# TimoLassmann/tagdust

Hardware: AMD Instinct MI355X
Metric: reads/s (150 bp, 8-barcode arch) (higher is better)
Workload: dtype f32

## Files before the change

tagdust_amd/csrc/td_jit.h:

```cpp
#pragma once
#include <string>
#include <vector>
#include "../../include/tagdust_hip.h"
#include "td_device.h"

#ifndef TD_HIDDEN
#define TD_HIDDEN __attribute__((visibility("hidden")))
#endif

struct TdSpecKnobs {
	int block = 512;
	int min_waves = 4;
	int lsum_oob = 1;
	int rt_min = 16;
	int groupcols = 18;
	int groupcols_fwd = 12;
	int prune = 1;
	int prune_sfx = 1;
	int restart = -1;
	int firstseg = -1;
	int trie_sh = 2;
	int profile = 0;
	int prune_stats = -1;
	std::string extra_opts;
};
TdSpecKnobs td_spec_knobs(void);

#define TD_PRUNE_TABLES 16
#define TD_PRUNE_RESTART_MAX 4

struct TdSpecPlan {
	TdSpecKnobs k;
	int S = 0, H = 0, C = 0;
	std::vector<int> col_off, hmm_off;
	std::vector<int> group, group_f;
	std::vector<int> pure_last, drop_m;
	std::vector<int> bw_off;
	int64_t halves = 0;
	std::vector<int> rt, rt_b;
	std::vector<int> base;
	std::vector<float> hi, lo, nv;
	bool trie_on = false;
	int trie_sh = 1, trie_n_share = 0;
	std::vector<int> trie_ord;
	int first_n = 0;
	int prune_segs = 0;
	int sfx_first = 0;
	float prune_z = 0.0f;
	int restart = 0;
};
TdSpecPlan td_spec_plan(const td_model_desc* m, const TdSpecKnobs& k);
TD_HIDDEN std::string td_spec_model_section(const td_model_desc* m, const TdSpecPlan& p, int lsum_oob, int window);

float td_spec_prune_z(const td_model_desc* m, int n_seg, int sfx_first);
void td_spec_prune_tables(const td_model_desc* m, const TdSpecPlan& p, int lcap, int stride, std::vector<float>& tab);
void td_spec_layout(TdSpecLayout& L, const TdSpecPlan& p, int lmax);
int td_spec_compile(const td_model_desc* m, const TdSpecPlan& p, int lsum_oob, int window, std::vector<char>& code, std::string& log,
                    uint64_t* key_out = nullptr, bool key_only = false);
int td_spec_compiles_started(void);
```

tagdust_amd/csrc/td_spec_kernel.inc:

```

#ifndef TDS_BLOCK
#define TDS_BLOCK 512
#endif
#ifndef TDS_MIN_WAVES
#define TDS_MIN_WAVES 4
#endif
#define TDS_REG_H 32
#define TDS_WPB (TDS_BLOCK / TD_WAVE)
#define NEG_INF (-__builtin_inff())
#define DEV __device__ __forceinline__

#define MODE_GET_LABEL 1
#define MODE_ARCH_COMP 5
#define OUT_SUCCESS 0
#define OUT_ARCH_MISMATCH 1
#define OUT_TOO_SHORT 2
#define OUT_BAR_FINGER_NOT_FOUND 3
#define OUT_MATCHES_ARTIFACTS 5
#define OUT_LOW_COMPLEXITY 6
#define N_OUTCOME_SLOTS 8
#define TDS_DIAG(k) (N_OUTCOME_SLOTS + 256 + ((k) - 192))

#ifndef TDS_LSUM_OOB
#define TDS_LSUM_OOB 1
// ... 131 lines not shown
}

#ifndef TDS_PROFILE
#define TDS_PROFILE 0
#endif
#define TDS_PHASE(k) do { if (TDS_PROFILE) { const long long t_ = (long long)__builtin_readcyclecounter(); \
	if (lane == 0) atomicAdd(&ka.counters[TDS_DIAG(240 + (k))], (unsigned long long)(t_ - tprof)); tprof = t_; } } while (0)

#ifndef TDS_WINDOW
#define TDS_WINDOW 0
#endif
constexpr bool kMaskDP = TD_H - kFirstN <= TDS_REG_H;

struct Wv {
	uint32_t* pmask;
	int nwm;
	uint8_t* slot;
	int lane, len, lmax, tmax, tmin;
	float* bm;
	uint8_t* ba;
	int cut;
	int cutS;
	const float* wa;
	const float* wb;
	int sstop;
	int sstopS;
	const float* wc;
	const float* wd;
	mutable int bad;
	bool rb_on, rf_on;
	float* rs;
	float* hb;
	int rWf;
	int rW;
	const float* bwt;
	const float* fbs;
	unsigned long long* stats;
	long long* tprof;
	const float* ptab;
	int pstride;
	const float* qr;
	const float* pr;
};

#ifndef TDS_LATE_CS
#define TDS_LATE_CS 1
#endif
#ifndef TDS_PF_DIST
#define TDS_PF_DIST 4
#endif
#ifndef TDS_PF_COLS
#define TDS_PF_COLS 2
#endif
#ifndef TDS_LDP
#define TDS_LDP 2
#endif
#ifndef TDS_LDT
#define TDS_LDT 4
#endif
#ifndef TDS_SCAN_B
#define TDS_SCAN_B 8
#endif
#ifndef TDS_PRUNE_TT
#define TDS_PRUNE_TT (-88.0f)
#endif
#ifndef TDS_PRUNE_MARGIN
#define TDS_PRUNE_MARGIN 1
#endif
#ifndef TDS_PRUNE_BGAP
#define TDS_PRUNE_BGAP 5.0f
#endif
#ifndef TDS_PRUNE_STATS
#define TDS_PRUNE_STATS 0
#endif

constexpr int cmin(int a, int b) { return a < b ? a : b; }
constexpr int pf_dist(int cols, bool rt) { return (!rt && cols <= TDS_PF_COLS) ? TDS_PF_DIST : 1; }
template <int D> struct IC { static constexpr int v = D; };
constexpr bool label_leading(int h)
{
	for (int j = 0; j < kPruneSegs; j++) if (h >= kHmmOff[j] && h < kHmmOff[j] + kNHmm[j]) return true;
	return false;
}
template <int PD, int D, typename F>
DEV void ring_block(F& step, const int base)
{
	if constexpr (D < PD) { step(IC<D>{}, base + D); ring_block<PD, D + 1>(step, base); }
}
template <int PD, int D, typename F>
DEV void ring_rest(F& step, const int base, const int iend)
{
	if constexpr (D < PD - 1) { if (base + D <= iend) { step(IC<D>{}, base + D); ring_rest<PD, D + 1>(step, base, iend); } }
}

template <int J, bool RT>
DEV void bwd_row(const int fa, const float (&Mn)[kNCol[J]], const float (&In)[kNCol[J]], const float Pn,
                 const BaseMask& kc, const int c, const BaseMask& kx, const int xi, SV (&Mc)[kNCol[J]], SV (&Ic)[kNCol[J]])
{
#define EM(gcol, mask, xval) (RT ? emit_rt(kBase[colr + (gcol)], kHi[J], kLo[J], kNv[J], mask, xval) : EMIT_M(col0 + (gcol), mask))
	constexpr int NC = kNCol[J];
	constexpr int K = NC - 1;
	const int col0 = kColOff[J] + (RT ? 0 : fa) * NC;
	const int colr = kColOff[J] + fa * NC;
	(void)colr;
	SV Dp = sv_none();
	{
		const int q = col0 + K;
		const SV M = addc(sv(Pn), kCols[q].t[7]);
		SV I = addc(sv(Pn), kCols[q].t[8]);
		I = lsum(I, addv(addc(sv(Mn[K]), kCols[q].t[4]), EM(K, kc, c)));
		I = lsum(I, addv(addc(sv(In[K]), kCols[q].t[3]), EMIT_I(q, kc)));
		Mc[K] = M; Ic[K] = I;
	}
#pragma unroll
	for (int g = K - 1; g >= 0; --g) {
		const int q = col0 + g;
		const float epc = EM(g + 1, kc, c);
		const float eic = EMIT_I(q, kc);
		SV M = addc(addv(sv(Mn[g + 1]), epc), kCols[q].t[0]);
		SV I = addv(addc(sv(In[g]), kCols[q].t[3]), eic);
		lsum2(M, addc(sv(Pn), kCols[q].t[7]), I, addc(sv(Pn), kCols[q].t[8]));
		lsum2(M, addc(addv(sv(In[g]), eic), kCols[q].t[1]), I, addv(addc(sv(Mn[g + 1]), kCols[q].t[4]), epc));
		SV D = addc(Dp, kCols[q].t[5]);
		lsum2(M, addc(Dp, kCols[q].t[2]), D, addc(addv(Mc[g + 1], EM(g + 1, kx, xi)), kCols[q].t[6]));
		Mc[g] = M; Ic[g] = I; Dp = D;
	}
#undef EM
}

template <int J, bool RT, int GT, int GB>
DEV void bwd_cols(const int fa, const float (&Mn)[kNCol[J]], const float (&In)[kNCol[J]], const float Pn,
                  const BaseMask& kc, const int c, const BaseMask& kx, const int xi, SV (&Mc)[kNCol[J]], SV (&Ic)[kNCol[J]], SV& Dp)
{
#define EM(gcol, mask, xval) (RT ? emit_rt(kBase[colr + (gcol)], kHi[J], kLo[J], kNv[J], mask, xval) : EMIT_M(col0 + (gcol), mask))
	constexpr int NC = kNCol[J];
	constexpr int K = NC - 1;
	const int col0 = kColOff[J] + (RT ? 0 : fa) * NC;
	const int colr = kColOff[J] + fa * NC;
	(void)colr;
	if constexpr (GT == K) {
		const int q = col0 + K;
		const SV M = addc(sv(Pn), kCols[q].t[7]);
		SV I = addc(sv(Pn), kCols[q].t[8]);
		I = lsum(I, addv(addc(sv(Mn[K]), kCols[q].t[4]), EM(K, kc, c)));
		I = lsum(I, addv(addc(sv(In[K]), kCols[q].t[3]), EMIT_I(q, kc)));
		Mc[K] = M; Ic[K] = I;
		Dp = sv_none();
	}
#pragma unroll
	for (int g = (GT == K ? K - 1 : GT); g >= GB; --g) {
		const int q = col0 + g;
		const float epc = EM(g + 1, kc, c);
		const float eic = EMIT_I(q, kc);
		SV M = addc(addv(sv(Mn[g + 1]), epc), kCols[q].t[0]);
		SV I = addv(addc(sv(In[g]), kCols[q].t[3]), eic);
		lsum2(M, addc(sv(Pn), kCols[q].t[7]), I, addc(sv(Pn), kCols[q].t[8]));
		lsum2(M, addc(addv(sv(In[g]), eic), kCols[q].t[1]), I, addv(addc(sv(Mn[g + 1]), kCols[q].t[4]), epc));
		SV D = addc(Dp, kCols[q].t[5]);
		lsum2(M, addc(Dp, kCols[q].t[2]), D, addc(addv(Mc[g + 1], EM(g + 1, kx, xi)), kCols[q].t[6]));
		Mc[g] = M; Ic[g] = I; Dp = D;
	}
#undef EM
}

#ifndef TDS_RESTART
#define TDS_RESTART 0
// ... 579 lines not shown
		}
		hi0 = fminf(hi0 + (__logf((float)(t > 1 ? t : 1)) + 0.02f), w.fbs[t]);
	}
	float Mlo[NC], Mhi[NC], Ilo[NC], Ihi[NC];
#pragma unroll
	for (int g = 0; g < NC; g++) { Mlo[g] = NEG_INF; Ilo[g] = NEG_INF; Mhi[g] = hi0; Ihi[g] = hi0; }
	int gc = 0;
	int closed_at = -1;
	auto close_check = [&](const int steps_done) __attribute__((always_inline)) {
		if (gc < NC) {
			bool cl = true;
#pragma unroll
			for (int g = 0; g < NC; g++) if (g == gc) cl = same(si(Mlo[g], Mhi[g])) && same(si(Ilo[g], Ihi[g]));
			if (__builtin_amdgcn_ballot_w64(!cl) == 0) { gc++; if (gc == NC) closed_at = steps_done; }
		}
	};
	int c_n = codes[q_lo * TD_WAVE + w.lane];
	float Pm_n = P[(q_lo - 1) * TD_WAVE + w.lane];
	for (int i = q_lo; i < q_hi; ++i) {
		const int c = c_n;
		const float Pm = Pm_n;
		{
			const int ip = (i + 1 < q_hi) ? i + 1 : i;
			c_n = codes[ip * TD_WAVE + w.lane];
			Pm_n = P[(ip - 1) * TD_WAVE + w.lane];
		}
		close_check(i - q_lo); close_check(i - q_lo);
		fstair_dispatch<J, 0>(gc, Mlo, Mhi, Ilo, Ihi, Pm, mk_mask(c));
	}
	close_check(q_hi - q_lo); close_check(q_hi - q_lo);
	if (gc < NC) w.bad |= 32;
	if (TDS_PRUNE_STATS && w.lane == 0) {
		const int st = closed_at >= 0 ? closed_at : q_hi - q_lo;
		atomicAdd(&w.stats[TDS_DIAG(194)], (unsigned long long)st); atomicAdd(&w.stats[TDS_DIAG(195)], 1ull);
		atomicMax(&w.stats[TDS_DIAG(192)], (unsigned long long)st);
	}
	float* rs = w.rs + (int64_t)kColOff[J] * 2 * TD_WAVE + w.lane;
#pragma unroll
	for (int g = 0; g < NC; g++) { rs[(2 * g) * TD_WAVE] = Mlo[g]; rs[(2 * g + 1) * TD_WAVE] = Ilo[g]; }
}

template <int J, int NF, bool RT>
DEV void fwd_group(const Wv& w, const uint8_t* __restrict__ codes, const float* __restrict__ P,
                   float* __restrict__ Cs, const float* __restrict__ PB, const uint8_t* __restrict__ BW,
                   float* __restrict__ DP, float* __restrict__ TOTAL, const float b, const int f0)
{
	const bool first = (f0 == 0);
#define EM(gcol, mask, xval) (RT ? emit_rt(kBase[colr + (gcol)], kHi[J], kLo[J], kNv[J], mask, xval) : EMIT_M(col0 + (gcol), mask))
	constexpr int NC = kNCol[J];
	constexpr int K = NC - 1;
	constexpr bool pure = kPureLast[J] != 0;
	constexpr int NS = NC - kPureLast[J];
	constexpr int DM = kDropM[J];
	constexpr int NSF = NS - DM;
	constexpr int ROWH = 2 * NS - DM;
	constexpr int NQ = NSF / 2;
	constexpr int NT = NSF & 1;
	constexpr bool skip_live = LIVE(kSkip[J]);
	float Mp[NF][NC], Ip[NF][NC], tot[NF];
#pragma unroll
	for (int f = 0; f < NF; f++) {
		tot[f] = NEG_INF;
#pragma unroll
		for (int g = 0; g < NC; g++) { Mp[f][g] = NEG_INF; Ip[f][g] = NEG_INF; }
	}
	if (TDS_RESTART && J >= kSfxFirst && w.rf_on) {
		const float* rs = w.rs + (int64_t)kColOff[J] * 2 * TD_WAVE + w.lane;
#pragma unroll
		for (int g = 0; g < NC; g++) { Mp[0][g] = rs[(2 * g) * TD_WAVE]; Ip[0][g] = rs[(2 * g + 1) * TD_WAVE]; }
	}
	constexpr bool p_init = (J == 0);
	const bool resumed = TDS_RESTART && (J >= kSfxFirst) && w.rf_on;
	const int i0 = resumed ? w.sstop - (TD_S - 1 - J) * (w.rWf + 1) : 1;
	float Pm = p_init ? 0.0f : P[(i0 - 1) * TD_WAVE + w.lane];
	constexpr int PD = pf_dist(NF * NC, RT);
	const int pmax = (w.tmax >= 1) ? w.tmax : 1;
	int c_q[PD];
	float Pi_q[PD], cs_q[PD], pb_q[PD], bm_q[PD], ik_q[PD][NF];
	int ba_q[PD];
	float MB_q[PD][NF][NSF + 1], IB_q[PD][NF][NSF + 1];
	constexpr bool pb_init = (J == TD_S - 1);
#define PBR(pos) (pb_init ? (((pos) == w.len + 1) ? 0.0f : NEG_INF) : PB[(pos) * TD_WAVE + w.lane])
#define BWROW(f_, pos_) (BW + ((int64_t)kBwOff[kHmmOff[J] + f0 + (f_)] * w.lmax + (int64_t)((pos_) - 1) * ROWH) * (TD_WAVE * 4))
#define TDS_FWD_FILL(d, p_raw) { \
		const int p_ = ((p_raw) <= pmax) ? (p_raw) : pmax; \
		c_q[d] = codes[p_ * TD_WAVE + w.lane]; \
		Pi_q[d] = p_init ? NEG_INF : P[p_ * TD_WAVE + w.lane]; \
		if (!first) cs_q[d] = Cs[p_ * TD_WAVE + w.lane]; \
		if (pure) pb_q[d] = PBR(p_ + 1); \
		if (own_sum && !first) { bm_q[d] = w.bm[p_ * TD_WAVE + w.lane]; ba_q[d] = w.ba[p_ * TD_WAVE + w.lane]; } \
		const bool rows_ = !((J >= kSfxFirst) && p_ < w.sstop);    \
_Pragma("unroll") \
		for (int f = 0; f < NF; f++) { \
			if (DM && rows_) ik_q[d][f] = ld1(BWROW(f, p_) + NSF * (TD_WAVE * 8), w.lane); \
			if (PD > 1 && rows_) { \
_Pragma("unroll") \
				for (int q = 0; q < NQ; q++) { \
					MB_q[d][f][2 * q] = ldk(BWROW(f, p_) + q * (TD_WAVE * 16), w.lane, 16, 0); IB_q[d][f][2 * q] = ldk(BWROW(f, p_) + q * (TD_WAVE * 16), w.lane, 16, 1); \
					MB_q[d][f][2 * q + 1] = ldk(BWROW(f, p_) + q * (TD_WAVE * 16), w.lane, 16, 2); IB_q[d][f][2 * q + 1] = ldk(BWROW(f, p_) + q * (TD_WAVE * 16), w.lane, 16, 3); \
				} \
				if (NT) { MB_q[d][f][NSF - 1] = ldk(BWROW(f, p_) + NQ * (TD_WAVE * 16), w.lane, 8, 0); IB_q[d][f][NSF - 1] = ldk(BWROW(f, p_) + NQ * (TD_WAVE * 16), w.lane, 8, 1); } \
			} \
		} \
	}
	constexpr bool own_sum = (J == 0) && (kFirstN > 0);
	float lacc[NF];
	uint32_t mbits[NF];
#pragma unroll
	for (int f = 0; f < NF; f++) { lacc[f] = 0.0f; mbits[f] = 0u; }
#pragma unroll
	for (int d = 0; d < PD; d++) {
		cs_q[d] = NEG_INF; pb_q[d] = 0.0f; bm_q[d] = -1.0f; ba_q[d] = 0;
#pragma unroll
		for (int f = 0; f < NF; f++) ik_q[d][f] = NEG_INF;
		TDS_FWD_FILL(d, i0 + d)
	}

	const int iend = (J < kPruneSegs && w.cut < w.tmax) ? w.cut : w.tmax;
	const int itail = (J == kPruneSegs && kPruneSegs > 0) ? w.cut + 1 : w.tmax + 1;
	(void)itail;
	if (i0 > 1 && kMaskDP && !own_sum) {
#pragma unroll
		for (int f = 0; f < NF; f++) {
			if (w.lane == 0) for (int wd = 0; wd < ((i0 - 1) >> 5); wd++) w.pmask[(kHmmOff[J] + f0 + f) * w.nwm + wd] = 0u;
			mbits[f] = 0u;
		}
	}
	auto step_cs = [&](auto dtag, auto cstag, const int i) __attribute__((always_inline)) {
		constexpr int d_ = decltype(dtag)::v;
		constexpr bool want_cs = decltype(cstag)::v != 0;
		const int c = c_q[d_];
		const float Pi = Pi_q[d_];
		const float pb = pb_q[d_];
		SV cs; cs.v = cs_q[d_]; cs.z = RT ? false : first;
		float bm = bm_q[d_];
		int ba = ba_q[d_];
		f32x4 cb[NF][NQ + 1];
		f32x2 ct[NF];
		const bool sfx_skip = (J >= kSfxFirst) && i < w.sstop;
		float ik[NF];
#pragma unroll
		for (int f = 0; f < NF; f++) {
			if constexpr (PD == 1) {
				const uint8_t* bw = BW + ((int64_t)kBwOff[kHmmOff[J] + f0 + f] * w.lmax + (int64_t)(i - 1) * ROWH) * (TD_WAVE * 4);
				if (!sfx_skip) {
#pragma unroll
					for (int p = 0; p < NQ; p++) cb[f][p] = ld4(bw + p * (TD_WAVE * 16), w.lane);
					if (NT) ct[f] = ld2(bw + NQ * (TD_WAVE * 16), w.lane);
				}
			} else {
#pragma unroll
				for (int p = 0; p < NQ; p++) cb[f][p] = f32x4{ MB_q[d_][f][2 * p], IB_q[d_][f][2 * p], MB_q[d_][f][2 * p + 1], IB_q[d_][f][2 * p + 1] };
				if (NT) ct[f] = f32x2{ MB_q[d_][f][NSF - 1], IB_q[d_][f][NSF - 1] };
			}
			ik[f] = ik_q[d_][f];
		}
		TDS_FWD_FILL(d_, i + PD)
		const int dn_ = (d_ + 1) % PD;
		const int c_n = c_q[dn_];
		const float pb_n = pb_q[dn_];
		float ik_n[NF];
#pragma unroll
		for (int f = 0; f < NF; f++) ik_n[f] = ik_q[dn_][f];
		float lpost[NF];
#pragma unroll
		for (int f = 0; f < NF; f++) lpost[f] = NEG_INF;
		const bool tail = (J == kPruneSegs && kPruneSegs > 0) && i >= itail;
		if (i <= w.len) {
			const SV PmS = sv(tail ? NEG_INF : Pm);
			const SV PiS = sv(tail ? NEG_INF : Pi);
			const BaseMask kc = mk_mask(c);
#pragma unroll
			for (int f = 0; f < NF; f++) {
				const int col0 = kColOff[J] + (RT ? 0 : (f0 + f)) * NC;
				const int colr = kColOff[J] + (f0 + f) * NC;
				(void)colr;
				const int h = kHmmOff[J] + f0 + f;
				SV Mc[NC], Ic[NC];
				SV Dc = sv_none();
				const float ei0 = EMIT_I(col0, kc);
				{
					const int q = col0;
					const SV M = addv(addc(PmS, kCols[q].sM), EM(0, kc, c));
					SV I = addc(PmS, kCols[q].sI);
					if (tail && LIVE(kCols[q].sI)) {
						if (!(Ip[f][0] + kCols[q].t[3] >= uload(w.wa, i))) w.bad |= 1;
					}
					I = lsum(I, addc(sv(Ip[f][0]), kCols[q].t[3]));
					I = lsum(I, addc(sv(Mp[f][0]), kCols[q].t[1]));
					I = addv(I, ei0);
					if (want_cs) { cs = lsum(cs, addc(M, kCols[q].t[7])); cs = lsum(cs, addc(I, kCols[q].t[8])); }
					Mc[0] = M; Ic[0] = I;
				}
#pragma unroll
				for (int g = 1; g <= K; ++g) {
					const int q = col0 + g, qp = q - 1;
					SV M = addc(PmS, kCols[q].sM);
					SV I = addc(PmS, kCols[q].sI);
					lsum2(M, addc(sv(Mp[f][g - 1]), kCols[qp].t[0]), I, addc(sv(Ip[f][g]), kCols[q].t[3]));
					lsum2(M, addc(sv(Ip[f][g - 1]), kCols[qp].t[4]), I, addc(sv(Mp[f][g]), kCols[q].t[1]));
					SV D = addc(Mc[g - 1], kCols[qp].t[2]);
					lsum2(M, addc(Dc, kCols[qp].t[6]), D, addc(Dc, kCols[qp].t[5]));
					M = addv(M, EM(g, kc, c));
					I = addv(I, EMIT_I(q, kc));
					if (want_cs) { cs = lsum(cs, addc(M, kCols[q].t[7])); cs = lsum(cs, addc(I, kCols[q].t[8])); }
					Mc[g] = M; Ic[g] = I; Dc = D;
				}
				if (tail && skip_live) { if (!(cs.v >= uload(w.wb, i))) w.bad |= 2; }
				if (want_cs) cs = lsum(cs, addc(PiS, kSkip[J]));
				if (!sfx_skip) {
				float MB[NC], IB[NC];
#pragma unroll
				for (int p = 0; p < NQ; p++) {
					const f32x4 v = cb[f][p];
					MB[2 * p] = v.x; IB[2 * p] = v.y; MB[2 * p + 1] = v.z; IB[2 * p + 1] = v.w;
				}
				if (NT) { MB[NSF - 1] = ct[f].x; IB[NSF - 1] = ct[f].y; }
				if constexpr (DM != 0) {
					constexpr int g = K - 1;
					const int q = col0 + g;
					const bool nxt = i < w.len;
					const int cx = (i < w.tmax) ? c_n : 0;
					const BaseMask kn = mk_mask(cx);
					SV MnK = addc(sv(pb_n), kCols[col0 + K].t[7]);
					if (!MnK.z) MnK.v = nxt ? MnK.v : NEG_INF;
					const float InK = nxt ? ik_n[f] : NEG_INF;
					SV Mr = addc(addv(MnK, EM(K, kn, cx)), kCols[q].t[0]);
					Mr = lsum(Mr, addc(sv(pb), kCols[q].t[7]));
					Mr = lsum(Mr, addc(addv(sv(InK), EMIT_I(q, kn)), kCols[q].t[1]));
					MB[g] = Mr.v; IB[g] = ik[f];
				}
				if (pure) {
					MB[K] = pb + kCols[col0 + K].t[7];
					IB[K] = pb + kCols[col0 + K].t[8];
				}
				constexpr bool want_tt = kNHmm[J] > 1;
				SV acc = sv_none(), tt = sv(tot[f]);
#pragma unroll
				for (int g = 0; g <= K; ++g) {
					const SV pm = subv(addv(Mc[g], MB[g]), b);
					if (want_tt && g == 0) tt = lsum(tt, pm);
					acc = lsum(acc, pm);
					if (want_tt && g == 0) tt = lsum(tt, subv(addv(addv(addc(PmS, kCols[col0].sI), ei0), IB[0]), b));
					acc = lsum(acc, subv(addv(Ic[g], IB[g]), b));
				}
				if (want_tt) tot[f] = tt.v;
				if (own_sum) {
					lacc[f] = post_prob(acc.v) + lacc[f];
					if (lacc[f] > bm) { bm = lacc[f]; ba = h; }
				} else if (kMaskDP) {
					lpost[f] = acc.v;
				} else {
					DP[((int64_t)(i - 1) * TD_H + h) * TD_WAVE + w.lane] = post_prob(acc.v);
				}
				}
#pragma unroll
				for (int g = 0; g < NC; g++) { Mp[f][g] = Mc[g].v; Ip[f][g] = Ic[g].v; }
			}
			if (want_cs) Cs[i * TD_WAVE + w.lane] = cs.v;
			if (own_sum) { w.bm[i * TD_WAVE + w.lane] = bm; w.ba[i * TD_WAVE + w.lane] = (uint8_t)ba; }
		}
		if (kMaskDP && !own_sum) {
#pragma unroll
			for (int f = 0; f < NF; f++) {
				const bool on = lpost[f] > -103.98f;
				const bool any_on = __builtin_amdgcn_ballot_w64(on) != 0;
				if (any_on) {
					float pp = 0.0f;
					if (on) pp = (float)exp((double)lpost[f]);
					if (i <= w.len) DP[((int64_t)(i - 1) * TD_H + kHmmOff[J] + f0 + f) * TD_WAVE + w.lane] = pp;
				}
				mbits[f] |= (any_on ? 1u : 0u) << ((i - 1) & 31);
				if ((((i - 1) & 31) == 31) || i == iend) {
					if (w.lane == 0) w.pmask[(kHmmOff[J] + f0 + f) * w.nwm + ((i - 1) >> 5)] = mbits[f];
					mbits[f] = 0u;
				}
			}
		}
		Pm = Pi;
	};
	{
		constexpr bool cs_late = TDS_LATE_CS && (J == TD_S - 1) && !((J == kPruneSegs && kPruneSegs > 0) && skip_live);
		auto step = [&](auto dtag, const int i) __attribute__((always_inline)) { step_cs(dtag, IC<1>{}, i); };
		auto step_nocs = [&](auto dtag, const int i) __attribute__((always_inline)) { step_cs(dtag, IC<0>{}, i); };
		int base = i0;
		if constexpr (cs_late) {
			const int i_cs = (w.tmin < iend) ? w.tmin : iend;
			for (; base + PD - 1 < i_cs; base += PD) ring_block<PD, 0>(step_nocs, base);
		}
		for (; base + PD - 1 <= iend; base += PD) ring_block<PD, 0>(step, base);
		ring_rest<PD, 0>(step, base, iend);
	}
	if (J < kPruneSegs && iend < w.tmax) {
		if (kMaskDP && !own_sum && w.lane == 0) {
#pragma unroll
			for (int f = 0; f < NF; f++)
				for (int wd = ((iend - 1) >> 5) + 1; wd < w.nwm; wd++) w.pmask[(kHmmOff[J] + f0 + f) * w.nwm + wd] = 0u;
		}
		if (kNHmm[J] > 1 && w.len > iend) {
#pragma unroll
			for (int f = 0; f < NF; f++) if (!(tot[f] >= TDS_PRUNE_TT)) w.bad |= 4;
		}
	}
	if (kNHmm[J] > 1) {
#pragma unroll
		for (int f = 0; f < NF; f++) TOTAL[(kHmmOff[J] + f0 + f) * TD_WAVE + w.lane] = tot[f];
	}
#undef EM
#undef PBR
#undef BWROW
#undef TDS_FWD_FILL
}

template <int J, int F0>
DEV void fwd_groups(const Wv& w, const uint8_t* __restrict__ codes, const float* __restrict__ P,
                    float* __restrict__ Cs, const float* __restrict__ PB, const uint8_t* __restrict__ BW,
                    float* __restrict__ DP, float* __restrict__ TOTAL, const float b)
{
	if constexpr (TDS_RESTART && F0 == 0 && J >= kSfxFirst) {
		if (w.rf_on) {
			const int q_hi = w.sstop - (TD_S - 1 - J) * (w.rWf + 1);
			fwd_stair<J>(w, codes, P, q_hi - w.rWf, q_hi);
		}
	}
	if constexpr (F0 == 0 && kRt[J] > 0) {
		for (int f0 = 0; f0 < kRt[J]; f0 += kGroupF[J]) fwd_group<J, kGroupF[J], true>(w, codes, P, Cs, PB, BW, DP, TOTAL, b, f0);
		fwd_groups<J, kRt[J]>(w, codes, P, Cs, PB, BW, DP, TOTAL, b);
	} else if constexpr (F0 < kNHmm[J]) {
		constexpr int NF = cmin(kGroupF[J], kNHmm[J] - F0);
		fwd_group<J, NF, false>(w, codes, P, Cs, PB, BW, DP, TOTAL, b, F0);
		fwd_groups<J, F0 + NF>(w, codes, P, Cs, PB, BW, DP, TOTAL, b);
	}
}

template <int J>
DEV void fwd_segments(const Wv& w, const uint8_t* __restrict__ codes, float* __restrict__ SF, const float* __restrict__ SB,
                      int rowlen, const uint8_t* __restrict__ BW, float* __restrict__ DP, float* __restrict__ TOTAL, const float b)
{
	if constexpr (J < TD_S) {
		fwd_groups<J, 0>(w, codes, SF + (int64_t)J * rowlen, SF + (int64_t)(J + 1) * rowlen, SB + (int64_t)(J + 1) * rowlen,
		                 BW, DP, TOTAL, b);
		if (TDS_PROFILE == 2 && J < 8) { const long long t_ = (long long)__builtin_readcyclecounter(); if (w.lane == 0) atomicAdd(&w.stats[TDS_DIAG(216 + J)], (unsigned long long)(t_ - *w.tprof)); *w.tprof = t_; }
		fwd_segments<J + 1>(w, codes, SF, SB, rowlen, BW, DP, TOTAL, b);
	}
}

constexpr bool path_word_trivial(int k)
{
	for (int b = 0; b < 4; b++) {
		const int v = kFirstN + 4 * k + b;
		if (v < TD_H && (kPredFirst[v] != 0 || kPredOff2[v + 1] != kPredOff2[v])) return false;
	}
	return true;
}
constexpr uint32_t path_word_identity(int k)
{
	uint32_t w = 0;
	for (int b = 0; b < 4; b++) w |= (uint32_t)((kFirstN + 4 * k + b) & 0xFF) << (8 * b);
	return w;
}

DEV int prune_scan(const float thr, const int len, const int tmax, const float* __restrict__ fbt, const float* __restrict__ bwt)
{
	int cl = 1;
	for (int i0 = 2; i0 <= tmax; i0 += TDS_SCAN_B) {
		float g[TDS_SCAN_B];
#pragma unroll
		for (int k = 0; k < TDS_SCAN_B; k++) {
			const int i = i0 + k;
			const int mm = (i <= len) ? len - i : 0;
			g[k] = bwt[mm];
		}
		__builtin_amdgcn_sched_barrier(0);
// ... 396 lines not shown
		}

		float Q;
		{
			float pbest = lsum(f_score, r_score);
			const double t = ((double)bar_prob + (double)f_score) - (double)pbest;
			const float tf = (float)t;
			const float e = (tf == NEG_INF) ? 0.0f : (float)exp((double)tf);
			pbest = (float)(1.0 - (double)e);
			if (pbest == 0.0f) Q = 40.0f;
			else if (pbest == 1.0f) Q = 0.0f;
			else Q = (float)(-10.0 * log10((double)pbest));
		}
		if (dead || len < 1) Q = 0.0f;

#define BMROW(pos) ((kPruneSegs > 0 && (pos) > w.cut) ? w.cut : (pos))
		int read_type = 0, barcode = -1, fingerprint = -1;
		const int nw1 = ka.nw1;
		uint32_t* keep = ka.out_keep + (int64_t)tile * nw1 * TD_WAVE;

		if (ka.mode == MODE_GET_LABEL) {
			int8_t* labels = ka.out_labels + (int64_t)tile * (ka.out_lmax + 1) * TD_WAVE;
			constexpr int F1 = kFirstN;
			constexpr int HL = H - F1;
			constexpr int PWL = (HL + 3) / 4;
			TDS_PHASE(3);
			if constexpr (HL <= TDS_REG_H) {
				float acc[HL];
	#pragma unroll
				for (int v = 0; v < HL; v++) acc[v] = 0.0f;
				constexpr int LD = TDS_LDP;
				float dq[LD][HL];
				uint32_t mq[LD];
				uint32_t mw[HL];
				auto mask_words = [&](const int word) __attribute__((always_inline)) {
					uint32_t t[HL];
#pragma unroll
					for (int v = 0; v < HL; v++) t[v] = w.pmask[(F1 + v) * w.nwm + word];
					__builtin_amdgcn_sched_barrier(0);
#pragma unroll
					for (int v = 0; v < HL; v++) mw[v] = (uint32_t)__builtin_amdgcn_readfirstlane((int)t[v]);
				};
#pragma unroll
				for (int v = 0; v < HL; v++) mw[v] = 0xFFFFFFFFu;
				if (kMaskDP && tmax >= 1) mask_words(0);
				const int rmax = (tmax >= 1) ? tmax - 1 : 0;
				auto request = [&](auto dtag, auto leadtag, const int p) __attribute__((always_inline)) {
					constexpr int d = decltype(dtag)::v;
					constexpr bool with_lead = decltype(leadtag)::v != 0;
					const int nb = p - 1;
					if (kMaskDP && (nb & 31) == 0 && nb > 0 && nb < tmax) mask_words(nb >> 5);
					const int row = (nb < rmax) ? nb : rmax;
					const float* dpn = DP + ((int64_t)row * H + F1) * TD_WAVE + lane;
					uint32_t bits = 0;
#pragma unroll
					for (int v = 0; v < HL; v++) {
						if (with_lead || !label_leading(F1 + v)) {
							dq[d][v] = dpn[v * TD_WAVE];
							bits |= ((mw[v] >> (nb & 31)) & 1u) << v;
						} else {
							dq[d][v] = 0.0f;
						}
					}
					mq[d] = (nb < tmax) ? bits : 0u;
				};
#pragma unroll
				for (int d = 0; d < LD; d++) mq[d] = 0u;
				float bm_p = 0.0f;
				int ba_p = 0;
				float bm_q[LD];
				int ba_q[LD];
				auto request_bm = [&](auto dtag, const int p) __attribute__((always_inline)) {
					constexpr int d = decltype(dtag)::v;
					if (F1 > 0) {
						const int pc = (p <= tmax) ? p : (tmax >= 1 ? tmax : 1);
						const int rb = BMROW(pc);
						bm_q[d] = w.bm[rb * TD_WAVE + lane]; ba_q[d] = w.ba[rb * TD_WAVE + lane];
					} else {
						bm_q[d] = 0.0f; ba_q[d] = 0;
					}
				};
				auto fill0 = [&](auto dtag, const int p) __attribute__((always_inline)) { request(dtag, IC<1>{}, p); request_bm(dtag, p); };
				ring_block<LD, 0>(fill0, 1);
				auto dp_step = [&](auto dtag, auto leadtag, auto reqtag, const int i) __attribute__((always_inline)) {
					constexpr int d = decltype(dtag)::v;
					float dc[HL];
#pragma unroll
					for (int v = 0; v < HL; v++) dc[v] = dq[d][v];
					const uint32_t mc = mq[d];
					const float bm_c = bm_q[d];
					const int ba_c = ba_q[d];
					if (decltype(reqtag)::v) { request(dtag, leadtag, i + LD); request_bm(dtag, i + LD); }
					uint32_t pws[PWL > 0 ? PWL : 1];
#pragma unroll
					for (int k = 0; k < PWL; k++) pws[k] = 0u;
					if (i <= len) {
						uint32_t pw = 0;
	#pragma unroll
						for (int v = HL - 1; v >= 0; v--) {
							float m = -1.0f;
							int mv = 0;
							if (F1 > 0 && kPredFirst[F1 + v]) {
								const bool gt = bm_p > m;
								m = gt ? bm_p : m;
								mv = gt ? ba_p : mv;
							}
	#pragma unroll
							for (int p = kPredOff2[F1 + v]; p < kPredOff2[F1 + v + 1]; p++) {
								const int u = kPredIdx2[p] - F1;
								const bool gt = acc[u] > m;
								m = gt ? acc[u] : m;
								mv = gt ? u + F1 : mv;
							}
							const bool st = acc[v] >= m;
							m = st ? acc[v] : m;
							mv = st ? v + F1 : mv;
							acc[v] = (((mc >> v) & 1u) ? dc[v] : 0.0f) + m;
							pw |= (uint32_t)mv << (8 * (v & 3));
							if ((v & 3) == 0) { pws[v >> 2] = pw; pw = 0; }
						}
					}
					uint32_t* pathi = PATH + (int64_t)(i - 1) * PWL * TD_WAVE + lane;
#pragma unroll
					for (int k = 0; k < PWL; k++) if (!path_word_trivial(k)) pathi[k * TD_WAVE] = pws[k];
					bm_p = bm_c; ba_p = ba_c;
				};
				{
					auto step_a = [&](auto dtag, const int i) __attribute__((always_inline)) { dp_step(dtag, IC<1>{}, IC<1>{}, i); };
					auto step_b = [&](auto dtag, const int i) __attribute__((always_inline)) { dp_step(dtag, IC<0>{}, IC<1>{}, i); };
					auto step_r = [&](auto dtag, const int i) __attribute__((always_inline)) { dp_step(dtag, IC<0>{}, IC<0>{}, i); };
					int base = 1;
					for (; base + LD - 1 <= tmax && (kPruneSegs == 0 || base + LD <= w.cut); base += LD) ring_block<LD, 0>(step_a, base);
					for (; base + LD - 1 <= tmax; base += LD) ring_block<LD, 0>(step_b, base);
					ring_rest<LD, 0>(step_r, base, tmax);
				}
				TDS_PHASE(4);
				{
					float m = -1.0f;
					int move = 0;
					if (F1 > 0 && len >= 1) {
						const float bl = w.bm[BMROW(len) * TD_WAVE + lane];
						if (bl > m) { m = bl; move = w.ba[BMROW(len) * TD_WAVE + lane]; }
					}
	#pragma unroll
					for (int v = 0; v < HL; v++) {
						const bool gt = acc[v] > m;
						m = gt ? acc[v] : m;
						move = gt ? v + F1 : move;
					}
					if (len >= 1) labels[len * TD_WAVE + lane] = (int8_t)move;
					constexpr int LDT = TDS_LDT;
					uint32_t wq[LDT][PWL > 0 ? PWL : 1];
					auto request_path = [&](auto dtag, const int r) __attribute__((always_inline)) {
						constexpr int d = decltype(dtag)::v;
						const int rc = (r >= 0) ? r : 0;
#pragma unroll
						for (int k = 0; k < PWL; k++)
							wq[d][k] = path_word_trivial(k) ? path_word_identity(k) : PATH[((int64_t)rc * PWL + k) * TD_WAVE + lane];
					};
					auto tb_step = [&](auto dtag, auto reqtag, const int r) __attribute__((always_inline)) {
						constexpr int d = decltype(dtag)::v;
						uint32_t wc[PWL > 0 ? PWL : 1];
#pragma unroll
						for (int k = 0; k < PWL; k++) wc[k] = wq[d][k];
						if (decltype(reqtag)::v) request_path(dtag, r - LDT);
						const int i = r + 1;
						if (i <= len) {
							if (move >= F1) {
								const int ml = move - F1;
								uint32_t pwv = wc[0];
	#pragma unroll
								for (int k = 1; k < PWL; k++) pwv = ((ml >> 2) == k) ? wc[k] : pwv;
								move = (pwv >> (8 * (ml & 3))) & 0xFF;
							}
							labels[(i - 1) * TD_WAVE + lane] = (int8_t)move;
						}
					};
					if (tmax >= 1) {
						auto fillp = [&](auto dtag, const int nr) __attribute__((always_inline)) { request_path(dtag, -nr); };
						auto step_w = [&](auto dtag, const int nr) __attribute__((always_inline)) { tb_step(dtag, IC<1>{}, -nr); };
						auto step_r = [&](auto dtag, const int nr) __attribute__((always_inline)) { tb_step(dtag, IC<0>{}, -nr); };
						int nbase = -(tmax - 1);
						ring_block<LDT, 0>(fillp, nbase);
						for (; nbase + LDT - 1 <= 0; nbase += LDT) ring_block<LDT, 0>(step_w, nbase);
						ring_rest<LDT, 0>(step_r, nbase, 0);
					}
				}

			} else {
				float* const ACCB = (float*)(w.slot + lay.acc);
				uint8_t* PATH8 = (uint8_t*)PATH;
				for (int v = 0; v < HL; v++) ACCB[v * TD_WAVE + lane] = 0.0f;
				float bm_p = 0.0f;
				int ba_p = 0;
				for (int i = 1; i <= tmax; i++) {
					if (i <= len) {
						const float* __restrict__ a0 = ACCB + (int64_t)((i - 1) & 1) * HL * TD_WAVE + lane;
						float* __restrict__ a1 = ACCB + (int64_t)(i & 1) * HL * TD_WAVE + lane;
						const float* __restrict__ dpi = DP + ((int64_t)(i - 1) * H + F1) * TD_WAVE + lane;
						uint8_t* __restrict__ pathi = PATH8 + (int64_t)(i - 1) * HL * TD_WAVE + lane;
						constexpr int CH = 8;
						for (int r = 0; r < kNRuns; r++) {
							const int v0 = kRunOff[r], v1 = kRunOff[r + 1];
							float m0 = -1.0f;
							int mv0 = 0;
							if (F1 > 0 && kPredFirst[F1 + v0]) {
								const bool gt = bm_p > m0;
								m0 = gt ? bm_p : m0;
								mv0 = gt ? ba_p : mv0;
							}
							const int p1 = kPredOff2[F1 + v0 + 1];
							for (int p = kPredOff2[F1 + v0]; p < p1; p += CH) {
								float au[CH];
								int uu[CH];
	#pragma unroll
								for (int k = 0; k < CH; k++) {
// ... 313 lines not shown
```

tagdust_amd/csrc/td_spec_plan.cpp:

```cpp
#include <math.h>
#include <stdio.h>
#include <stdlib.h>
#include <string.h>

#include <map>
#include <string>
#include <vector>

#include "td_jit.h"

static std::string flit(float v)
{
	if (isinf(v)) return v < 0 ? "(-__builtin_inff())" : "__builtin_inff()";
	if (v != v) return "__builtin_nanf(\"\")";
	char buf[64];
	snprintf(buf, sizeof buf, "%af", (double)v);
	return buf;
}

TdSpecKnobs td_spec_knobs(void)
{
	TdSpecKnobs k;
	auto num = [](const char* name, int unset) { const char* e = getenv(name); return e ? atoi(e) : unset; };
	auto flag = [](const char* name, int unset) -> int { const char* e = getenv(name); return e ? atoi(e) != 0 : unset; };
	if (const int v = num("TD_SPEC_BLOCK", 0); v >= 64 && v <= 1024 && v % 64 == 0) k.block = v;
	if (const int v = num("TD_SPEC_MINWAVES", 0); v >= 1 && v <= 8) k.min_waves = v;
	if (const int v = num("TD_SPEC_GROUPCOLS", 0); v > 0) k.groupcols = v;
	k.groupcols_fwd = num("TD_SPEC_GROUPCOLS_FWD", k.groupcols_fwd);
	k.rt_min = num("TD_SPEC_RT_MIN", k.rt_min);
	k.trie_sh = num("TD_SPEC_TRIE_SH", k.trie_sh);
	k.profile = num("TD_SPEC_PROFILE", k.profile);
	k.lsum_oob = flag("TD_SPEC_LSUM_OOB", k.lsum_oob);
	k.prune = flag("TD_SPEC_PRUNE", k.prune);
	k.prune_sfx = flag("TD_SPEC_PRUNE_SFX", k.prune_sfx);
	k.restart = flag("TD_SPEC_RESTART", k.restart);
	k.firstseg = flag("TD_SPEC_FIRSTSEG", k.firstseg);
	k.prune_stats = flag("TD_SPEC_PRUNE_STATS", k.prune_stats);
	if (const char* e = getenv("TD_SPEC_EXTRA_OPTS")) k.extra_opts = e;
	return k;
}

namespace {
int pure_last(const td_model_desc* m, int j, int col_off)
{
	for (int f = 0; f < m->n_hmm[j]; f++) {
		const int q = col_off + f * m->n_col[j] + m->n_col[j] - 1;
		if (!(m->trans[q * 9 + 4] == -INFINITY) || !(m->trans[q * 9 + 3] == -INFINITY)) return 0;
	}
	return 1;
}

int rt_prefix(const td_model_desc* m, int j, int col_off, int* base , float* hi, float* lo, float* nv, int min_hmms)
{
	const int n = m->n_hmm[j], nc = m->n_col[j];
	if (n < min_hmms) return 0;
	auto match_type = [&](int q, int* b, float* h, float* l, float* v) -> bool {
		const float* e = m->eM + (size_t)q * 5;
		for (int x = 0; x < 4; x++) {
			const float other = e[(x + 1) & 3];
			bool ok = !(e[x] == other);
			for (int y = 0; y < 4 && ok; y++) if (y != x && !(e[y] == other)) ok = false;
			if (ok) { *b = x; *h = e[x]; *l = other; *v = e[4]; return true; }
		}
		return false;
	};
	int b0; float h0, l0, v0;
	if (!match_type(col_off, &b0, &h0, &l0, &v0)) return 0;
	int f = 0;
	for (; f < n; f++) {
		bool ok = true;
		for (int g = 0; g < nc && ok; g++) {
			const int q = col_off + f * nc + g, q0 = col_off + g;
			if (memcmp(m->trans + (size_t)q * 9, m->trans + (size_t)q0 * 9, 36) || memcmp(m->eI + (size_t)q * 5, m->eI + (size_t)q0 * 5, 20) ||
			    memcmp(&m->sM[q], &m->sM[q0], 4) || memcmp(&m->sI[q], &m->sI[q0], 4)) { ok = false; break; }
			int b; float h, l, v;
			if (!match_type(q, &b, &h, &l, &v) || memcmp(&h, &h0, 4) || memcmp(&l, &l0, 4) || memcmp(&v, &v0, 4)) { ok = false; break; }
			base[q] = b;
		}
		if (!ok) break;
	}
	*hi = h0; *lo = l0; *nv = v0;
	return f >= min_hmms ? f : 0;
}

int group_size(int n_hmm, int n_col, int target)
{
	int maxf = target / n_col;
	if (maxf < 1) maxf = 1;
	if (maxf > n_hmm) maxf = n_hmm;
	const int groups = (n_hmm + maxf - 1) / maxf;
	return (n_hmm + groups - 1) / groups;
}

int first_labels(const td_model_desc* m, int firstseg)
{
	const int H = m->H, n0 = m->n_hmm[0];
	const int mode = firstseg >= 0 ? firstseg : H > 32;
	if (!mode) return 0;
	if (n0 < 2 || n0 >= H) return 0;
	for (int v = 0; v < n0; v++)
		for (int u = 0; u < v; u++) if (m->A[u * H + v] == 1.0f) return 0;
	for (int w = n0; w < H; w++) {
		int c = 0;
		for (int u = 0; u < n0; u++) c += m->A[u * H + w] == 1.0f;
		if (c != 0 && c != n0) return 0;
	}
	return n0;
}

bool read_like(const td_model_desc* m, int j, int co)
{
	if (m->n_hmm[j] != 1 || m->n_col[j] != 1) return false;
	const float* t = m->trans + (size_t)co * 9;
	for (int k = 0; k < 9; k++) if (k != TD_II && k != TD_ISKIP && t[k] > -INFINITY) return false;
	return m->sM[co] == -INFINITY && m->sI[co] > -INFINITY && t[TD_II] > -INFINITY && t[TD_ISKIP] > -INFINITY;
}
}

TdSpecPlan td_spec_plan(const td_model_desc* m, const TdSpecKnobs& k)
// ... 88 lines not shown
	s += buf;
	snprintf(buf, sizeof buf, "#define TD_S %d\n#define TD_H %d\n#define TD_C %d\n#define TD_REQ_FINGER %d\n", S, H, C, req);
	s += buf;
	s += "struct GCol { float t[9]; float sM, sI; float eM[5]; float eI[5]; };\n";
	auto int_array = [&](const char* name, const std::vector<int>& v) {
		s += std::string("static constexpr int ") + name + "[" + std::to_string(v.size()) + "] = {";
		for (size_t i = 0; i < v.size(); i++) { s += std::to_string(v[i]); if (i + 1 < v.size()) s += ","; }
		s += "};\n";
	};
	int_array("kNHmm", std::vector<int>(m->n_hmm, m->n_hmm + S)); int_array("kNCol", std::vector<int>(m->n_col, m->n_col + S));
	int_array("kColOff", p.col_off); int_array("kHmmOff", p.hmm_off);
	int_array("kRtB", p.rt_b);
	s += std::string("static constexpr bool kTrieOn = ") + (p.trie_on ? "true" : "false") + ";\n";
	s += "static constexpr int kTrieSH = " + std::to_string(p.trie_sh) + ";\n";
	s += "static constexpr int kTrieNShare = " + std::to_string(p.trie_n_share) + ";\n";
	int_array("kTrieOrd", p.trie_ord);
	int_array("kGroup", p.group); int_array("kGroupF", p.group_f); int_array("kPureLast", p.pure_last); int_array("kDropM", p.drop_m); int_array("kBwOff", p.bw_off);
	int_array("kRt", p.rt); int_array("kBase", p.base);
	auto float_array = [&](const char* name, const std::vector<float>& v) {
		s += std::string("static constexpr float ") + name + "[" + std::to_string(v.size()) + "] = {";
		for (size_t i = 0; i < v.size(); i++) { s += flit(v[i]); if (i + 1 < v.size()) s += ","; }
		s += "};\n";
	};
	float_array("kHi", p.hi); float_array("kLo", p.lo); float_array("kNv", p.nv);
	s += "static constexpr float kSkip[" + std::to_string(S) + "] = {";
	for (int j = 0; j < S; j++) { s += flit(m->skip[j]); if (j + 1 < S) s += ","; }
	s += "};\n";
	s += "static constexpr float kBg[5] = {";
	for (int i = 0; i < 5; i++) { s += flit(m->bg[i]); if (i < 4) s += ","; }
	s += "};\n";
	const float stay_arg = (float)(1.0 - (1.0 / (double)(float)m->avg_len));
	const float exit_arg = (float)(1.0 / (double)(float)m->avg_len);
	s += "static constexpr float kRStay = " + flit(stay_arg == 0.0f ? -INFINITY : (float)log((double)stay_arg)) + ";\n";
	s += "static constexpr float kRExit = " + flit(exit_arg == 0.0f ? -INFINITY : (float)log((double)exit_arg)) + ";\n";
	s += "static constexpr GCol kCols[" + std::to_string(C) + "] = {\n";
	for (int k = 0; k < C; k++) {
		s += " {{";
		for (int t = 0; t < 9; t++) { s += flit(m->trans[k * 9 + t]); if (t < 8) s += ","; }
		s += "}," + flit(m->sM[k]) + "," + flit(m->sI[k]) + ",{";
		for (int e = 0; e < 5; e++) { s += flit(m->eM[k * 5 + e]); if (e < 4) s += ","; }
		s += "},{";
		for (int e = 0; e < 5; e++) { s += flit(m->eI[k * 5 + e]); if (e < 4) s += ","; }
		s += "}},\n";
	}
	s += "};\n";
	s += "static constexpr unsigned kHinfo[" + std::to_string(H) + "] = {";
	for (int h = 0; h < H; h++) {
		const int seg = m->label[h] & 0xFFFF, f = (m->label[h] >> 16) & 0x7FFF;
		unsigned v = (unsigned)(unsigned char)m->seg_type[seg] | ((unsigned)seg << 8) | ((unsigned)f << 16);
		if (m->seg_type[seg] == 'B' && f == m->n_hmm[seg] - 1) v |= 0x80000000u;
		snprintf(buf, sizeof buf, "0x%08xu%s", v, h + 1 < H ? "," : "");
		s += buf;
	}
	s += "};\n";
	std::vector<int> poff(H + 1, 0), pidx;
	for (int v = 0; v < H; v++) {
		poff[v] = (int)pidx.size();
		for (int u = 0; u < v; u++) if (m->A[u * H + v] == 1.0f) pidx.push_back(u);
	}
	poff[H] = (int)pidx.size();
	if (pidx.empty()) pidx.push_back(0);
	int_array("kPredOff", poff); int_array("kPredIdx", pidx);
	const int first_n = p.first_n;
	std::vector<int> pfirst(H, 0), poff2(H + 1, 0), pidx2;
	for (int v = 0; v < H; v++) {
		poff2[v] = (int)pidx2.size();
		for (int i = poff[v]; i < poff[v + 1]; i++) {
			if (pidx[i] < first_n) pfirst[v] = 1; else pidx2.push_back(pidx[i]);
		}
	}
	poff2[H] = (int)pidx2.size();
	if (pidx2.empty()) pidx2.push_back(0);
	s += "static constexpr int kFirstN = " + std::to_string(first_n) + ";\n";
	int_array("kPredFirst", pfirst); int_array("kPredOff2", poff2); int_array("kPredIdx2", pidx2);
	std::vector<int> runs;
	for (int v = first_n; v < H; v++) {
		bool same = v > first_n && pfirst[v] == pfirst[v - 1] && poff2[v + 1] - poff2[v] == poff2[v] - poff2[v - 1];
		for (int k = 0; same && k < poff2[v + 1] - poff2[v]; k++) same = pidx2[poff2[v] + k] == pidx2[poff2[v - 1] + k];
		if (!same) runs.push_back(v - first_n);
	}
	runs.push_back(H - first_n);
	s += "static constexpr int kPruneSegs = " + std::to_string(p.prune_segs) + ";\n";
	s += "static constexpr int kSfxFirst = " + std::to_string(p.sfx_first) + ";\n";
	s += "static constexpr float kPruneZ = " + flit(p.prune_z) + ";\n";
	if (p.k.prune_stats >= 0) s += std::string("#define TDS_PRUNE_STATS ") + (p.k.prune_stats ? "1" : "0") + "\n";
	s += std::string("#ifndef TDS_RESTART\n#define TDS_RESTART ") + (p.restart ? "1" : "0") + "\n#endif\n";
	s += "static constexpr int kNRuns = " + std::to_string((int)runs.size() - 1) + ";\n";
	int_array("kRunOff", runs);
	return s;
}

void td_spec_layout(TdSpecLayout& L, const TdSpecPlan& p, int lmax)
{
	auto al = [](int64_t v) { return (v + 255) & ~(int64_t)255; };
	int64_t o = 0;
	L.codes = o; o = al(o + (int64_t)(lmax + 2) * TD_WAVE);
	L.sb = o;    o = al(o + (int64_t)(p.S + 1) * (lmax + 2) * TD_WAVE * 4);
	L.sf = o;    o = al(o + (int64_t)(p.S + 1) * (lmax + 2) * TD_WAVE * 4);
	L.bw = o;    o = al(o + p.halves * lmax * TD_WAVE * 4 + 1024);
	L.dp = o;    o = al(o + (int64_t)lmax * p.H * TD_WAVE * 4);
	L.path = o;  o = al(o + (int64_t)lmax * ((p.H + 3) / 4) * TD_WAVE * 4);
	L.total = o; o = al(o + (int64_t)p.H * TD_WAVE * 4);
	L.rs = o;    o = al(o + (int64_t)2 * p.C * TD_WAVE * 4);
	L.bm = o;    o = al(o + (int64_t)(lmax + 2) * TD_WAVE * 4);
	L.ba = o;    o = al(o + (int64_t)(lmax + 2) * TD_WAVE);
	L.acc = o;   o = al(o + (int64_t)2 * p.H * TD_WAVE * 4);
	L.pmask = o; o = al(o + (int64_t)p.H * ((lmax + 31) / 32) * 4);
	L.slot_bytes = o;
}
```

Measured before the change: 83.14 million.

## Specialize forward tail and Viterbi DP steps past the prune cut window

Adds a default-on 'quiet' mode. In the forward pass of the first post-prune segment, steps beyond the cut use a compile-time tail variant that skips loading and using the predecessor P values. In the Viterbi/path DP, steps past the cut window skip the max-over-predecessors search for label-leading states when their predecessors lie outside the segment, writing a fixed backpointer instead. This removes loads and compare work in long read tails, at the cost of more template instantiations, larger code and register pressure.

```diff
diff --git a/tagdust_amd/csrc/td_jit.h b/tagdust_amd/csrc/td_jit.h
--- a/tagdust_amd/csrc/td_jit.h
+++ b/tagdust_amd/csrc/td_jit.h
@@ -19,6 +19,7 @@
 	int prune_sfx = 1;
 	int restart = -1;
 	int firstseg = -1;
+	int quiet = 1;
 	int trie_sh = 2;
 	int profile = 0;
 	int prune_stats = -1;
diff --git a/tagdust_amd/csrc/td_spec_kernel.inc b/tagdust_amd/csrc/td_spec_kernel.inc
--- a/tagdust_amd/csrc/td_spec_kernel.inc
+++ b/tagdust_amd/csrc/td_spec_kernel.inc
@@ -237,6 +237,21 @@
 	for (int j = 0; j < kPruneSegs; j++) if (h >= kHmmOff[j] && h < kHmmOff[j] + kNHmm[j]) return true;
 	return false;
 }
+#ifndef TDS_QUIET
+#define TDS_QUIET kQuiet
+#endif
+constexpr bool quiet_labels_ok()
+{
+	for (int j = 0; j < kPruneSegs; j++)
+		for (int v = kHmmOff[j]; v < kHmmOff[j] + kNHmm[j]; v++)
+			for (int p = kPredOff[v]; p < kPredOff[v + 1]; p++) if (kPredIdx[p] >= kHmmOff[j]) return false;
+	return true;
+}
+#ifndef TDS_QUIET_FWD
+#define TDS_QUIET_FWD TDS_QUIET
+#endif
+constexpr bool kQuietFwd = TDS_QUIET_FWD != 0;
+constexpr bool kQuietDP = TDS_QUIET != 0 && kPruneSegs > 0 && kFirstN == 0 && TD_H <= TDS_REG_H && quiet_labels_ok();
 template <int PD, int D, typename F>
 DEV void ring_block(F& step, const int base)
 {
@@ -982,10 +997,10 @@
 	constexpr bool pb_init = (J == TD_S - 1);
 #define PBR(pos) (pb_init ? (((pos) == w.len + 1) ? 0.0f : NEG_INF) : PB[(pos) * TD_WAVE + w.lane])
 #define BWROW(f_, pos_) (BW + ((int64_t)kBwOff[kHmmOff[J] + f0 + (f_)] * w.lmax + (int64_t)((pos_) - 1) * ROWH) * (TD_WAVE * 4))
-#define TDS_FWD_FILL(d, p_raw) { \
+#define TDS_FWD_FILL(d, p_raw, NO_P_) { \
 		const int p_ = ((p_raw) <= pmax) ? (p_raw) : pmax; \
 		c_q[d] = codes[p_ * TD_WAVE + w.lane]; \
-		Pi_q[d] = p_init ? NEG_INF : P[p_ * TD_WAVE + w.lane]; \
+		if (!(NO_P_)) Pi_q[d] = p_init ? NEG_INF : P[p_ * TD_WAVE + w.lane]; \
 		if (!first) cs_q[d] = Cs[p_ * TD_WAVE + w.lane]; \
 		if (pure) pb_q[d] = PBR(p_ + 1); \
 		if (own_sum && !first) { bm_q[d] = w.bm[p_ * TD_WAVE + w.lane]; ba_q[d] = w.ba[p_ * TD_WAVE + w.lane]; } \
@@ -1013,7 +1028,7 @@
 		cs_q[d] = NEG_INF; pb_q[d] = 0.0f; bm_q[d] = -1.0f; ba_q[d] = 0;
 #pragma unroll
 		for (int f = 0; f < NF; f++) ik_q[d][f] = NEG_INF;
-		TDS_FWD_FILL(d, i0 + d)
+		TDS_FWD_FILL(d, i0 + d, false)
 	}
 
 	const int iend = (J < kPruneSegs && w.cut < w.tmax) ? w.cut : w.tmax;
@@ -1026,9 +1041,10 @@
 			mbits[f] = 0u;
 		}
 	}
-	auto step_cs = [&](auto dtag, auto cstag, const int i) __attribute__((always_inline)) {
+	auto step_cs = [&](auto dtag, auto cstag, auto tailtag, const int i) __attribute__((always_inline)) {
 		constexpr int d_ = decltype(dtag)::v;
 		constexpr bool want_cs = decltype(cstag)::v != 0;
+		constexpr bool tail_s = decltype(tailtag)::v != 0;
 		const int c = c_q[d_];
 		const float Pi = Pi_q[d_];
 		const float pb = pb_q[d_];
@@ -1055,7 +1071,7 @@
 			}
 			ik[f] = ik_q[d_][f];
 		}
-		TDS_FWD_FILL(d_, i + PD)
+		TDS_FWD_FILL(d_, i + PD, tail_s)
 		const int dn_ = (d_ + 1) % PD;
 		const int c_n = c_q[dn_];
 		const float pb_n = pb_q[dn_];
@@ -1065,10 +1081,10 @@
 		float lpost[NF];
 #pragma unroll
 		for (int f = 0; f < NF; f++) lpost[f] = NEG_INF;
-		const bool tail = (J == kPruneSegs && kPruneSegs > 0) && i >= itail;
+		const bool tail = tail_s || ((J == kPruneSegs && kPruneSegs > 0) && i >= itail);
 		if (i <= w.len) {
-			const SV PmS = sv(tail ? NEG_INF : Pm);
-			const SV PiS = sv(tail ? NEG_INF : Pi);
+			const SV PmS = tail_s ? sv_none() : sv(tail ? NEG_INF : Pm);
+			const SV PiS = tail_s ? sv_none() : sv(tail ? NEG_INF : Pi);
 			const BaseMask kc = mk_mask(c);
 #pragma unroll
 			for (int f = 0; f < NF; f++) {
@@ -1177,18 +1193,24 @@
 				}
 			}
 		}
-		Pm = Pi;
+		if (!tail_s) Pm = Pi;
 	};
 	{
 		constexpr bool cs_late = TDS_LATE_CS && (J == TD_S - 1) && !((J == kPruneSegs && kPruneSegs > 0) && skip_live);
-		auto step = [&](auto dtag, const int i) __attribute__((always_inline)) { step_cs(dtag, IC<1>{}, i); };
-		auto step_nocs = [&](auto dtag, const int i) __attribute__((always_inline)) { step_cs(dtag, IC<0>{}, i); };
+		constexpr bool tail_split = kQuietFwd && (J == kPruneSegs && kPruneSegs > 0);
+		auto step = [&](auto dtag, const int i) __attribute__((always_inline)) { step_cs(dtag, IC<1>{}, IC<0>{}, i); };
+		auto step_nocs = [&](auto dtag, const int i) __attribute__((always_inline)) { step_cs(dtag, IC<0>{}, IC<0>{}, i); };
+		auto step_t = [&](auto dtag, const int i) __attribute__((always_inline)) { step_cs(dtag, IC<1>{}, IC<1>{}, i); };
+		auto step_t_nocs = [&](auto dtag, const int i) __attribute__((always_inline)) { step_cs(dtag, IC<0>{}, IC<1>{}, i); };
+		(void)step_t; (void)step_t_nocs;
 		int base = i0;
 		if constexpr (cs_late) {
 			const int i_cs = (w.tmin < iend) ? w.tmin : iend;
-			for (; base + PD - 1 < i_cs; base += PD) ring_block<PD, 0>(step_nocs, base);
-		}
-		for (; base + PD - 1 <= iend; base += PD) ring_block<PD, 0>(step, base);
+			for (; base + PD - 1 < i_cs && (!tail_split || base < itail); base += PD) ring_block<PD, 0>(step_nocs, base);
+			if constexpr (tail_split) { for (; base + PD - 1 < i_cs && base + PD - 1 <= iend; base += PD) ring_block<PD, 0>(step_t_nocs, base); }
+		}
+		for (; base + PD - 1 <= iend && (!tail_split || base < itail); base += PD) ring_block<PD, 0>(step, base);
+		if constexpr (tail_split) { for (; base + PD - 1 <= iend; base += PD) ring_block<PD, 0>(step_t, base); }
 		ring_rest<PD, 0>(step, base, iend);
 	}
 	if (J < kPruneSegs && iend < w.tmax) {
@@ -1751,8 +1773,9 @@
 				};
 				auto fill0 = [&](auto dtag, const int p) __attribute__((always_inline)) { request(dtag, IC<1>{}, p); request_bm(dtag, p); };
 				ring_block<LD, 0>(fill0, 1);
-				auto dp_step = [&](auto dtag, auto leadtag, auto reqtag, const int i) __attribute__((always_inline)) {
+				auto dp_step = [&](auto dtag, auto leadtag, auto reqtag, auto quiettag, const int i) __attribute__((always_inline)) {
 					constexpr int d = decltype(dtag)::v;
+					constexpr bool quiet = decltype(quiettag)::v != 0;
 					float dc[HL];
 #pragma unroll
 					for (int v = 0; v < HL; v++) dc[v] = dq[d][v];
@@ -1767,6 +1790,11 @@
 						uint32_t pw = 0;
 	#pragma unroll
 						for (int v = HL - 1; v >= 0; v--) {
+							if (quiet && label_leading(F1 + v)) {
+								pw |= (uint32_t)(v + F1) << (8 * (v & 3));
+								if ((v & 3) == 0) { pws[v >> 2] = pw; pw = 0; }
+								continue;
+							}
 							float m = -1.0f;
 							int mv = 0;
 							if (F1 > 0 && kPredFirst[F1 + v]) {
@@ -1795,12 +1823,15 @@
 					bm_p = bm_c; ba_p = ba_c;
 				};
 				{
-					auto step_a = [&](auto dtag, const int i) __attribute__((always_inline)) { dp_step(dtag, IC<1>{}, IC<1>{}, i); };
-					auto step_b = [&](auto dtag, const int i) __attribute__((always_inline)) { dp_step(dtag, IC<0>{}, IC<1>{}, i); };
-					auto step_r = [&](auto dtag, const int i) __attribute__((always_inline)) { dp_step(dtag, IC<0>{}, IC<0>{}, i); };
+					auto step_a = [&](auto dtag, const int i) __attribute__((always_inline)) { dp_step(dtag, IC<1>{}, IC<1>{}, IC<0>{}, i); };
+					auto step_b = [&](auto dtag, const int i) __attribute__((always_inline)) { dp_step(dtag, IC<0>{}, IC<1>{}, IC<0>{}, i); };
+					auto step_q = [&](auto dtag, const int i) __attribute__((always_inline)) { dp_step(dtag, IC<0>{}, IC<1>{}, IC<1>{}, i); };
+					auto step_r = [&](auto dtag, const int i) __attribute__((always_inline)) { dp_step(dtag, IC<0>{}, IC<0>{}, IC<0>{}, i); };
+					(void)step_q;
 					int base = 1;
 					for (; base + LD - 1 <= tmax && (kPruneSegs == 0 || base + LD <= w.cut); base += LD) ring_block<LD, 0>(step_a, base);
-					for (; base + LD - 1 <= tmax; base += LD) ring_block<LD, 0>(step_b, base);
+					for (; base + LD - 1 <= tmax && (!kQuietDP || base < w.cut + kPruneSegs + 1); base += LD) ring_block<LD, 0>(step_b, base);
+					if constexpr (kQuietDP) { for (; base + LD - 1 <= tmax; base += LD) ring_block<LD, 0>(step_q, base); }
 					ring_rest<LD, 0>(step_r, base, tmax);
 				}
 				TDS_PHASE(4);
diff --git a/tagdust_amd/csrc/td_spec_plan.cpp b/tagdust_amd/csrc/td_spec_plan.cpp
--- a/tagdust_amd/csrc/td_spec_plan.cpp
+++ b/tagdust_amd/csrc/td_spec_plan.cpp
@@ -35,6 +35,7 @@
 	k.prune_sfx = flag("TD_SPEC_PRUNE_SFX", k.prune_sfx);
 	k.restart = flag("TD_SPEC_RESTART", k.restart);
 	k.firstseg = flag("TD_SPEC_FIRSTSEG", k.firstseg);
+	k.quiet = flag("TD_SPEC_QUIET", k.quiet);
 	k.prune_stats = flag("TD_SPEC_PRUNE_STATS", k.prune_stats);
 	if (const char* e = getenv("TD_SPEC_EXTRA_OPTS")) k.extra_opts = e;
 	return k;
@@ -289,6 +290,7 @@
 	runs.push_back(H - first_n);
 	s += "static constexpr int kPruneSegs = " + std::to_string(p.prune_segs) + ";\n";
 	s += "static constexpr int kSfxFirst = " + std::to_string(p.sfx_first) + ";\n";
+	s += "static constexpr int kQuiet = " + std::to_string(p.k.quiet ? 1 : 0) + ";\n";
 	s += "static constexpr float kPruneZ = " + flit(p.prune_z) + ";\n";
 	if (p.k.prune_stats >= 0) s += std::string("#define TDS_PRUNE_STATS ") + (p.k.prune_stats ? "1" : "0") + "\n";
 	s += std::string("#ifndef TDS_RESTART\n#define TDS_RESTART ") + (p.restart ? "1" : "0") + "\n#endif\n";
```

Result: faster. 84.36 million, median of 6 (+1.5%).
